# carlosnatalino/optical-rl-gym

Measured on AMD Instinct MI355X. Metric: env-steps/sec RMSA-v0 NSFNET batch 65536, higher is better.
Workload: dtype u64 bitmaps + f64 statistics

## Files before the change

optical_rl_gym_amd/csrc/orl_device_split.h:

```cpp
#pragma once
#include "orl_device_g8.h"

namespace orl {
namespace sp {

#define ORL_PROF_SLOTS 48
#define ORL_PROF_WAVES 16384
#ifdef ORL_TIMING
struct Prof { long long t; unsigned long long acc[ORL_PROF_SLOTS]; };
static __device__ unsigned long long g_prof[ORL_PROF_WAVES * ORL_PROF_SLOTS];
#define ORL_PROF_BEGIN_() do { for (int k_ = 0; k_ < ORL_PROF_SLOTS; k_++) prof.acc[k_] = 0; prof.t = clock64(); } while (0)
#define ORL_PROF_(k) do { long long n_ = clock64(); prof.acc[k] += (unsigned long long)(n_ - prof.t); prof.t = n_; } while (0)
#define ORL_PROF_END_() do { if ((threadIdx.x & 63) == 0) { const size_t w_ = ((size_t)blockIdx.x * (blockDim.x >> 6) + (threadIdx.x >> 6)) % ORL_PROF_WAVES; \
    unsigned long long* g_ = ::orl::sp::g_prof + w_ * ORL_PROF_SLOTS; \
    for (int k_ = 0; k_ < ORL_PROF_SLOTS; k_++) g_[k_] += prof.acc[k_]; } } while (0)
#define ORL_PROF_BEGIN() ORL_PROF_BEGIN_()
#define ORL_PROF_END() ORL_PROF_END_()
#define ORL_PROFA(k) ORL_PROF_(k)
#define ORL_PROF(k) ORL_PROF_(16 + (k))
#define ORL_PROFR(k) ORL_PROF_(32 + (k))
#else
struct Prof { long long t; };
#define ORL_PROF_BEGIN() do { } while (0)
#define ORL_PROF_END() do { } while (0)
#define ORL_PROFA(k) do { } while (0)
#define ORL_PROF(k) do { } while (0)
#define ORL_PROFR(k) do { } while (0)
#endif
#define ORL_PROFA_BEGIN() do { } while (0)
#define ORL_PROFA_END() do { } while (0)
#define ORL_PROFR_BEGIN() do { } while (0)
#define ORL_PROFR_END() do { } while (0)

struct Recip { double d, r; };
__device__ __forceinline__ Recip recip_of(double d) {
  Recip k;
  k.d = d;
  double r = __builtin_amdgcn_rcp(d);
  double e = __builtin_fma(-d, r, 1.0);
  r = __builtin_fma(r, e, r);
  e = __builtin_fma(-d, r, 1.0);
  k.r = __builtin_fma(r, e, r);
  return k;
}
__device__ __forceinline__ double div_by(double x, const Recip& k) {
  const double q = x * k.r;
  return __builtin_fma(__builtin_fma(-k.d, q, x), k.r, q);
}
__device__ __forceinline__ double div_pos(double x, double d) { return div_by(x, recip_of(d)); }

#include "orl_diag.h"
using g8::EnvG;
using g8::gballot;
using g8::gget;

struct Item { ulonglong2 a, b; };
__device__ __forceinline__ Item make_item(i64 env, u32 link, int nmask, u64 m0, u64 m1, u64 cores, int op) {
  Item it;
  it.a.x = (u64)(u32)env | ((u64)(link & 0xffu) << 32) | ((u64)(u32)nmask << 40) | ((u64)(u32)op << 44);
  it.a.y = m0;
  it.b.x = m1;
  it.b.y = cores;
  return it;
}
__device__ __forceinline__ void item_store(ulonglong2* q, size_t idx, const Item& it) { q[2 * idx] = it.a; q[2 * idx + 1] = it.b; }

__device__ __forceinline__ size_t wave_reserve(const DevParams& P, int cnt, u32* wave_counts, int lane) {
  const int grp = lane >> 3;
  int pre = 0, tot = 0;
#pragma unroll
  for (int g = 0; g < 8; g++) {
    const int c = __builtin_amdgcn_readlane(cnt, 8 * g);
    pre += (g < grp) ? c : 0;
    tot += c;
  }
  const size_t wave = (size_t)blockIdx.x * (blockDim.x >> 6) + (threadIdx.x >> 6);
  if (lane == 0) wave_counts[wave] = (u32)tot;
  return wave * (size_t)P.q_wave + (size_t)pre;
}

struct Mask2 { u64 lo, hi; int w0; };
__device__ __forceinline__ Mask2 mask2(int s0, int n) {
  Mask2 m;
  const int b = s0 & 63;
  const u64 ones = (1ull << n) - 1ull;
  m.w0 = s0 >> 6;
  m.lo = ones << b;
  m.hi = (b + n > 64) ? (ones >> (64 - b)) : 0ull;
  return m;
}
__device__ __forceinline__ u64 mask2_word(const Mask2& m, int w) { return (w == m.w0) ? m.lo : ((w == m.w0 + 1) ? m.hi : 0ull); }
__device__ __forceinline__ void row_apply_mask(u64* row, int s0, int n, bool provision) {
  const Mask2 m = mask2(s0, n);
  if (provision) {
    __hip_atomic_fetch_and(row + m.w0, ~m.lo, __ATOMIC_RELAXED, __HIP_MEMORY_SCOPE_WORKGROUP);
    if (m.hi) __hip_atomic_fetch_and(row + m.w0 + 1, ~m.hi, __ATOMIC_RELAXED, __HIP_MEMORY_SCOPE_WORKGROUP);
  } else {
    __hip_atomic_fetch_or(row + m.w0, m.lo, __ATOMIC_RELAXED, __HIP_MEMORY_SCOPE_WORKGROUP);
    if (m.hi) __hip_atomic_fetch_or(row + m.w0 + 1, m.hi, __ATOMIC_RELAXED, __HIP_MEMORY_SCOPE_WORKGROUP);
  }
}
template <bool CP> struct SinkEntryOf { typedef SinkEntry type; };
template <> struct SinkEntryOf<true> { typedef SinkEntryC type; };
#define ORL_EV_META(S0, N, T, PROV) ((u64)(u32)(S0) | ((u64)(u32)(N) << 9) | ((u64)(u32)(T) << 15) | ((u64)((PROV) ? 1u : 0u) << 24))
template <bool CP, bool RD = false> struct SinkT {
  typedef typename SinkEntryOf<CP>::type Entry;
  ulonglong2* ev;
  double ev_clock;
  int ev_at;
  int ev_rel0;
  int ev_t;
  unsigned short* list;
  u32* list_n;
  Entry* tab;
  u32* tally;
  int tw;
  unsigned short* mtab;
  int nrel;
  u64* rows;
  int roww;
  bool active;
  bool deferred;
  int cnt;
};
typedef SinkT<false> Sink;
__device__ __forceinline__ void sink_entry_clear(SinkEntry& t) { t.crn = 0ull; }
__device__ __forceinline__ void sink_entry_clear(SinkEntryC& t) { t.bits = 0u; }
__device__ __forceinline__ int sink_entry_add(SinkEntry* t, u64 m, int core, bool prov) {
  const u64 crn = t->crn | (prov ? (1ull << 44) : 0ull);
  const int j = (int)((crn >> 40) & 15);
  if (j < 4) t->mk0 = (j == 0 ? 0ull : t->mk0) | (m << (16 * j));
  else t->mk1 = (j == 4 ? 0ull : t->mk1) | (m << (16 * (j - 4)));
  t->crn = (crn & ((1ull << 44) | 0xffffffffffull)) | ((u64)(u32)core << (5 * j)) | ((u64)(u32)(j + 1) << 40);
  return j | (int)((crn >> 44) & 1) << 8;
}
template <bool CP, bool RD>
__device__ __forceinline__ void sink_add(SinkT<CP, RD>& s, const PathRec& rec, int core, int s0, int n, int lane, bool prov = false) {
  const int hops = path_rec_byte(rec, 0);
  if constexpr (RD) {
    u32 lm0 = 0u, lm1 = 0u;
    for (int h = lane & 7; h < hops; h += 8) {
      const int link = path_rec_byte(rec, 2 + h);
      row_apply_mask(s.rows + (size_t)link * s.roww, s0, n, prov);
      if (link < 32) lm0 |= 1u << link; else lm1 |= 1u << (link - 32);
    }
    lm0 |= (u32)dpp_i<ORL_DPP_XOR1>((int)lm0); lm1 |= (u32)dpp_i<ORL_DPP_XOR1>((int)lm1);
    lm0 |= (u32)dpp_i<ORL_DPP_XOR2>((int)lm0); lm1 |= (u32)dpp_i<ORL_DPP_XOR2>((int)lm1);
    lm0 |= (u32)dpp_i<ORL_DPP_HALF_MIRROR>((int)lm0); lm1 |= (u32)dpp_i<ORL_DPP_HALF_MIRROR>((int)lm1);
    if ((lane & 7) == 0) {
      s.ev[2 * s.ev_at] = make_ulonglong2(ORL_EV_META(s0, n, s.ev_t, prov), (u64)lm0 | ((u64)lm1 << 32));
      s.ev[2 * s.ev_at + 1] = make_ulonglong2((u64)__double_as_longlong(s.ev_clock), 0ull);
    }
  } else if constexpr (CP) {
    const int k = prov ? 0 : ++s.nrel;
    if ((lane & 7) == 0) s.mtab[k] = (unsigned short)((u32)s0 | ((u32)n << 9));
    for (int h = lane & 7; h < hops; h += 8) {
      const int link = path_rec_byte(rec, 2 + h);
      atomicOr(&s.tab[link].bits, 1u << k);
      if (s.rows) row_apply_mask(s.rows + (size_t)link * s.roww, s0, n, prov);
    }
  } else {
    const u64 m = (u64)(u32)s0 | ((u64)(u32)n << 9);
    for (int h = lane & 7; h < hops; h += 8) {
      const int r = sink_entry_add(s.tab + path_rec_byte(rec, 2 + h), m, core, prov);
      const int j = r & 15;
      s.cnt += (j == 0) ? 1 : 0;
      if (s.list && (j == 0 || (j == 1 && (r >> 8))))
        s.list[atomicAdd(s.list_n, 1u)] = (unsigned short)((j << 15) | (((lane >> 3) & 7) << 8) | path_rec_byte(rec, 2 + h));
    }
  }
}

__device__ __forceinline__ void emit_items(const DevParams& P, i64 env, const Sink& sink, bool any, int lane, ulonglong2* q, u32* counts) {
  const int gl = lane & 7, E = P.E;
  const int cnt = g8_sum(any ? sink.cnt : 0);
  const size_t base = wave_reserve(P, cnt, counts, lane);
  if (cnt) {
    size_t at = base;
    for (int l0 = 0; l0 < E; l0 += 8) {
      const int l = l0 + gl;
      const u64 crn = (l < E) ? sink.tab[l].crn : 0ull;
      const int nm = (int)((crn >> 40) & 15);
      const u32 fb = gballot(nm > 0, lane);
      if (nm > 0)
        item_store(q, at + __popc(fb & ((1u << gl) - 1u)),
                   make_item(env, (u32)l, nm, sink.tab[l].mk0, nm > 4 ? sink.tab[l].mk1 : 0ull, crn & 0xffffffffffull,
                             1 | (int)((crn >> 44) & 1) << 1));
      at += __popc(fb);
    }
  }
}

#define ORL_SVC_WIN 12
struct SvcBuf {
  double q, ht;
  u32 pk;
  int cnt;
};
__device__ __forceinline__ bool svc_empty(const SvcBuf& b) { return (b.cnt & 0xff) >= (b.cnt >> 8); }
struct SvcNext { double q, ht; u32 pk; };
__device__ __forceinline__ SvcNext svc_take(SvcBuf& b, int lane) {
  const int k = b.cnt & 0xff;
  SvcNext s;
  s.q = gget(b.q, k, lane);
  s.ht = gget(b.ht, k, lane);
  s.pk = gget(b.pk, k, lane);
  b.cnt += 1;
  return s;
}
__device__ __forceinline__ int svc_wrap(int i) { const u32 u = (u32)i, d = u - 624u; return (int)(d < u ? d : u); }
__device__ __forceinline__ int svc_choice(const double* cum, int n, double u) {
  const double x = u * (cum[n - 1] + 0.0);
  const int m = n - 1;
  if (m <= 0) return 0;
  int b = 0;
  if (m > 8 && m <= 72) {
    double p[8];
#pragma unroll
    for (int j = 0; j < 8; j++) p[j] = cum[8 * j + 7 < m ? 8 * j + 7 : m - 1];
#pragma unroll
    for (int j = 0; j < 8; j++) b += (8 * j + 7 < m && p[j] <= x) ? 1 : 0;
  } else if (m > 72) {
    int lo = 0, hi = m;
    while (lo < hi) {
      const int mid = (lo + hi) >> 1;
      if (cum[mid] <= x) lo = mid + 1; else hi = mid;
    }
    return lo;
  }
  double c[8];
#pragma unroll
  for (int k = 0; k < 8; k++) c[k] = cum[8 * b + k < m ? 8 * b + k : m - 1];
  int cnt = 8 * b;
#pragma unroll
  for (int k = 0; k < 8; k++) cnt += (8 * b + k < m && c[k] <= x) ? 1 : 0;
  return cnt;
}
template <int ENV>
__device__ __forceinline__ void svc_generate(const DevParams& P, u64* rec, u32* mt, const double2* rates_wave, int lane, int n_want,
                                             SvcBuf& sb, bool active) {
  const int gl = lane & 7;
  const bool seek = (ENV != ENV_RWA) && P.bit_rate_mode == 0;
  const int FIXED = (ENV == ENV_RWA) ? 8 : (P.bit_rate_mode == 0 ? 8 : 10);
  const u32 sh = 32u - (u32)P.rand_bits, rn = (u32)P.rand_n;
  const u64 idw = active ? rec[SC_ID_MTPOS] : 0ull;
  const int pos = (int)(idw >> 32);
  u32 cur[ORL_SVC_WIN], nxt[ORL_SVC_WIN], far[ORL_SVC_WIN];
#pragma unroll
  for (int k = 0; k < ORL_SVC_WIN; k++) {
    const int i0 = svc_wrap(pos + gl + 8 * k);
    cur[k] = active ? mt[i0] : 0u;
    nxt[k] = active ? mt[svc_wrap(i0 + 1)] : 0u;
    far[k] = active ? mt[svc_wrap(i0 + 397)] : 0u;
  }
  u32 nx[ORL_SVC_WIN];
  u32 acc0 = 0u, acc1 = 0u, acc2 = 0u;
#pragma unroll
  for (int k = 0; k < ORL_SVC_WIN; k++) {
    const u32 y = (cur[k] & 0x80000000u) | (nxt[k] & 0x7fffffffu);
    nx[k] = far[k] ^ (y >> 1) ^ ((y & 1u) ? 0x9908b0dfu : 0u);
    if (seek) {
      u32 t = cur[k];
      t ^= (t >> 11);
      t ^= (t << 7) & 0x9d2c5680u;
      t ^= (t << 15) & 0xefc60000u;
      t ^= (t >> 18);
      const u32 byte = gballot((t >> sh) < rn, lane);
      if (k < 4) acc0 |= byte << (8 * (k & 3));
      else if (k < 8) acc1 |= byte << (8 * (k & 3));
      else acc2 |= byte << (8 * (k & 3));
    }
  }
  int o = 0, my_o = 0, my_a = 0, got = 0;
  {
    const u64 m_lo = (u64)acc0 | ((u64)acc1 << 32);
    bool ok = active;
#pragma unroll
    for (int j = 0; j < 8; j++) {
      if (ok && j < n_want) {
        const int c = o + FIXED;
        int a = c - 1;
        if (seek) {
          const u64 xl = (c < 64) ? (m_lo >> c) : 0ull;
          const u32 xh = (c <= 64) ? acc2 : ((c < 8 * ORL_SVC_WIN) ? ((acc2 >> (c - 64)) << (c - 64)) : 0u);
          if (xl == 0ull && xh == 0u) ok = false;
          else a = (xl != 0ull) ? c + (int)__builtin_ctzll(xl) : 64 + (int)__builtin_ctz(xh);
        } else if (c > 8 * ORL_SVC_WIN) {
          ok = false;
        }
        if (ok) {
          if (gl == j) { my_o = o; my_a = a; }
          o = seek ? a + 1 : c;
          got = j + 1;
        }
      }
    }
  }
  const bool mine = active && gl < got;
  u32 w[10], wa = 0u;
#pragma unroll
  for (int t = 0; t < 10; t++) w[t] = (mine && t < FIXED) ? mt[svc_wrap(pos + my_o + t)] : 0u;
  if (seek && mine) wa = mt[svc_wrap(pos + my_a)];
#pragma unroll
  for (int k = 0; k < ORL_SVC_WIN; k++)
// ... 685 lines not shown
      int nd = 0, top = -1, h0 = 0x7fffffff, h1 = 0x7fffffff;
      const int hwm = e.ev_hwm;
      for (int base = gl, ord = 0; base < hwm; base += 8 * ORL_SCAN_BATCH, ord += ORL_SCAN_BATCH) {
        double tt[ORL_SCAN_BATCH];
#pragma unroll
        for (int k = 0; k < ORL_SCAN_BATCH; k++) {
          const int i = base + 8 * k;
          tt[k] = e.ev_time[i < hwm ? i : hwm - 1];
        }
        scan_batch_fence(tt);
#pragma unroll
        for (int k = 0; k < ORL_SCAN_BATCH; k++) {
          const int i = base + 8 * k;
          tt[k] = (i < hwm) ? tt[k] : INF;
        }
#pragma unroll
        for (int k = 0; k < ORL_SCAN_BATCH; k++) {
          const double t = tt[k];
          const int i = base + 8 * k;
          const bool due_t = t <= e.now;
          nd += due_t ? 1 : 0;
          const bool empty = (t == INF);
          top = empty ? top : i;
          h1 = (empty && h0 != 0x7fffffff && h1 == 0x7fffffff) ? i : h1;
          h0 = (empty && h0 == 0x7fffffff) ? i : h0;
          u32 q = (u32)__builtin_fmax(__builtin_fmin((t - e.now) * 4096.0 + 524288.0, 8388606.0), 0.0);
          q = empty ? 8388607u : q;
          q = (due_t && q > 524287u) ? 524287u : q;
          u32 x = (q << 8) | (u32)(ord + k);
#pragma unroll
          for (int j = 0; j <= NS; j++) {
            const u32 lo = kb[j] < x ? kb[j] : x;
            x = kb[j] < x ? x : kb[j];
            kb[j] = lo;
          }
        }
      }
      double bt[NS];
      int bi[NS];
#pragma unroll
      for (int k = 0; k < NS; k++) {
        const bool any = (kb[k] >> 8) < 8388607u;
        bi[k] = gl + 8 * (int)(kb[k] & 255u);
        bt[k] = any ? e.ev_time[bi[k]] : INF;
      }
      const u32 qn = kb[NS] >> 8;
      const double T_lane = (qn >= 8388607u) ? INF : (qn < 2u ? -INF : e.now + ((double)qn - 524290.0) * (1.0 / 4096.0));
      const double T = g8::g8_min(T_lane);
#pragma unroll
      for (int k = 0; k < NS; k++) { st[k] = (bt[k] < T || bt[k] <= e.now) ? bt[k] : INF; si[k] = bi[k]; }
      e.t_soon = T;
      dirty = (1 << NS) - 1;
      due_all = g8_sum(nd);
      e.ev_hwm = g8_max(top) + 1;
      {
        const bool v0 = h0 < e.ev_hwm, v1 = h1 < e.ev_hwm;
        const u32 b0 = gballot(v0, lane), b1 = gballot(v1, lane);
        unsigned short* fs = (unsigned short*)(e.scal + SC_FREE0);
        if (v0) fs[__popc(b0 & ((1u << gl) - 1u))] = (unsigned short)h0;
        if (v1) fs[__popc(b0) + __popc(b1 & ((1u << gl) - 1u))] = (unsigned short)h1;
        e.nfree = __popc(b0) + __popc(b1);
      }
      ORL_PROF(5);
    }
    int ndl = 0;
    double ct = INF;
    int ci = 0x7fffffff, ck = 0;
#pragma unroll
    for (int k = 0; k < NS; k++) {
      const bool due = st[k] <= e.now;
      ndl += due ? 1 : 0;
      if (due && (st[k] < ct || (st[k] == ct && si[k] < ci))) { ct = st[k]; ci = si[k]; ck = k; }
    }
    const int tot = g8_sum(ndl);
    if (tot == 0) {
      if (e.now < e.t_soon) break;
      if (round > 0 || due_all >= 0) {
        if (!sink.active) { ORL_DBG(8, 1); ORL_DBG(9, e.now < e.t_soon ? 0 : 1); ORL_DBG(10, due_all > 0 ? 1 : 0); sink.deferred = true; return; }
        break;
      }
      continue;
    }
    if (!sink.active) {
      const int total = due_all >= 0 ? due_all : tot;
      if constexpr (CP) {
        sink.active = total <= P.rel_limit;
      } else {
      sink.active = total + extra <= P.item_masks;
      if (!sink.active && total < 200) {
        for (int base = gl; base < e.ev_hwm; base += 64) {
          double tt[8];
#pragma unroll
          for (int k = 0; k < 8; k++) {
            const int i = base + 8 * k;
            const double v = e.ev_time[i < e.ev_hwm ? i : e.ev_hwm - 1];
            tt[k] = (i < e.ev_hwm) ? v : INF;
          }
#pragma unroll
          for (int k = 0; k < 8; k++) {
            if (tt[k] <= e.now) {
              const u64 info = e.ev_info[base + 8 * k];
              const PathRec rec = path_rec_load(P, (int)(info & 0xffffffu));
              const int hops = path_rec_byte(rec, 0);
              for (int h = 0; h < hops; h++) {
                const int link = path_rec_byte(rec, 2 + h);
                atomicAdd(sink.tally + (link >> 2), 1u << (8 * (link & 3)));
              }
            }
          }
        }
        wave_fence();
        u32 mx = 0;
        for (int wd = gl; wd < sink.tw; wd += 8) {
          const u32 v = sink.tally[wd];
          const u32 a0 = v & 0xff, a1 = (v >> 8) & 0xff, a2 = (v >> 16) & 0xff, a3 = v >> 24;
          u32 m01 = a0 > a1 ? a0 : a1, m23 = a2 > a3 ? a2 : a3;
          m01 = m01 > m23 ? m01 : m23;
          mx = mx > m01 ? mx : m01;
        }
        sink.active = g8_max((int)mx) <= P.item_masks;
      }
      }
      if (!sink.active) {
        ORL_DBG(11, 1);
        sink.deferred = true;
        return;
      }
    }
    if constexpr (CP) {
      u32 rk = 0u;
      int n_round = 0;
      if (e.rank_pairs && __ballot(ndl > 1) == 0ull) {
        int r = 1;
#define ORL_RANK_STEP(OT, OI) { const double ot_ = (OT); const int oi_ = (OI); \
                                r += (ot_ < ct || (ot_ == ct && oi_ < ci)) ? 1 : 0; \
                                if (ot_ < INF && gl == (oi_ & 7)) e.ev_time[oi_] = INF; }
        ORL_RANK_STEP(dpp_d<ORL_DPP_XOR1>(ct), dpp_i<ORL_DPP_XOR1>(ci))
        ORL_RANK_STEP(dpp_d<ORL_DPP_XOR2>(ct), dpp_i<ORL_DPP_XOR2>(ci))
        ORL_RANK_STEP(dpp_d<ORL_DPP_XOR3>(ct), dpp_i<ORL_DPP_XOR3>(ci))
        {
          const double mt = dpp_d<ORL_DPP_HALF_MIRROR>(ct);
          const int mi = dpp_i<ORL_DPP_HALF_MIRROR>(ci);
          ORL_RANK_STEP(mt, mi)
          ORL_RANK_STEP(dpp_d<ORL_DPP_XOR1>(mt), dpp_i<ORL_DPP_XOR1>(mi))
          ORL_RANK_STEP(dpp_d<ORL_DPP_XOR2>(mt), dpp_i<ORL_DPP_XOR2>(mi))
          ORL_RANK_STEP(dpp_d<ORL_DPP_XOR3>(mt), dpp_i<ORL_DPP_XOR3>(mi))
        }
#undef ORL_RANK_STEP
        n_round = tot;
        if (ndl == 1) {
          if (gl == (ci & 7)) e.ev_time[ci] = INF;
          rk = (u32)r << (6 * ck);
          dirty |= 1 << ck;
#pragma unroll
          for (int k = 0; k < NS; k++)
            if (k == ck) st[k] = INF;
        }
      } else {
        for (;;) {
          double bt = ct;
          int bi = ci, bl = gl;
#define ORL_MIN_STEP(CTRL) { double ot = dpp_d<CTRL>(bt); int oi = dpp_i<CTRL>(bi); int ol = dpp_i<CTRL>(bl); \
                             if (ot < bt || (ot == bt && oi < bi)) { bt = ot; bi = oi; bl = ol; } }
          ORL_MIN_STEP(ORL_DPP_XOR1) ORL_MIN_STEP(ORL_DPP_XOR2) ORL_MIN_STEP(ORL_DPP_HALF_MIRROR)
#undef ORL_MIN_STEP
          if (!(bt <= e.now)) break;
          n_round++;
          if (gl == (bi & 7)) e.ev_time[bi] = INF;
          if (gl == bl) {
            rk |= (u32)n_round << (6 * ck);
            dirty |= 1 << ck;
            ct = INF; ci = 0x7fffffff;
            int nk = 0;
#pragma unroll
            for (int k = 0; k < NS; k++) {
              if (k == ck) st[k] = INF;
              const bool due = st[k] <= e.now;
              if (due && (st[k] < ct || (st[k] == ct && si[k] < ci))) { ct = st[k]; ci = si[k]; nk = k; }
            }
            ck = nk;
          }
        }
      }
      ORL_PROF(6);
      int d_br = 0, d_nh = 0;
      const int nfree0 = e.nfree, nrel0 = sink.nrel;
      unsigned short* fs = (unsigned short*)(e.scal + SC_FREE0);
      while (rk) {
        const int k = (int)__builtin_ctz(rk) / 6;
        const int r = (int)((rk >> (6 * k)) & 63u);
        rk &= ~(63u << (6 * k));
        int idx = si[0];
#pragma unroll
        for (int j = 1; j < NS; j++) idx = (k == j) ? si[j] : idx;
        const u64 info = (idx == pushed_idx) ? pushed_info : ((idx == pre_idx) ? pre_info : e.ev_info[idx]);
        const PathRec rec = path_rec_load(P, (int)(info & 0xffffffu));
        const int s0 = (int)((info >> 24) & 0xfffu), n = (int)((info >> 36) & 0xffu), br = (int)((info >> 49) & 0x7fffu);
        const int hops = path_rec_byte(rec, 0), kk = nrel0 + r;
        if constexpr (RD) {
          u64 lm = 0ull;
          for (int h = 0; h < hops; h++) {
            const int link = path_rec_byte(rec, 2 + h);
            row_apply_mask(sink.rows + (size_t)link * sink.roww, s0, n, false);
            lm |= 1ull << link;
          }
          sink.ev[2 * (sink.ev_rel0 + kk - 1)] = make_ulonglong2(ORL_EV_META(s0, n, sink.ev_t, false), lm);
          sink.ev[2 * (sink.ev_rel0 + kk - 1) + 1] = make_ulonglong2((u64)__double_as_longlong(e.now), 0ull);
        } else {
        sink.mtab[kk] = (unsigned short)((u32)s0 | ((u32)n << 9));
        for (int h = 0; h < hops; h++) {
          const int link = path_rec_byte(rec, 2 + h);
          atomicOr(&sink.tab[link].bits, 1u << kk);
          if (sink.rows) row_apply_mask(sink.rows + (size_t)link * sink.roww, s0, n, false);
        }
        }
        const int fp = nfree0 + r - 1;
        if (fp < ORL_FREE_SLOTS) fs[fp] = (unsigned short)idx;
        d_br += br;
        d_nh += n * hops;
      }
      e.ev_cnt -= n_round;
      e.nfree = (nfree0 + n_round < ORL_FREE_SLOTS) ? nfree0 + n_round : ORL_FREE_SLOTS;
      sink.nrel = nrel0 + n_round;
      e.s_br -= (i64)g8_sum(d_br);
      e.s_nh -= (i64)g8_sum(d_nh);
    } else {
      u64 inf0 = 0;
      PathRec rc0 = PathRec();
      if (ci != 0x7fffffff) { inf0 = (ci == pushed_idx) ? pushed_info : ((ci == pre_idx) ? pre_info : e.ev_info[ci]); rc0 = path_rec_load(P, (int)(inf0 & 0xffffffu)); }
      ORL_PROF(6);
      for (;;) {
        double bt = ct;
        int bi = ci, bl = gl;
  #define ORL_MIN_STEP(CTRL) { double ot = dpp_d<CTRL>(bt); int oi = dpp_i<CTRL>(bi); int ol = dpp_i<CTRL>(bl); \
                               if (ot < bt || (ot == bt && oi < bi)) { bt = ot; bi = oi; bl = ol; } }
        ORL_MIN_STEP(ORL_DPP_XOR1) ORL_MIN_STEP(ORL_DPP_XOR2) ORL_MIN_STEP(ORL_DPP_HALF_MIRROR)
  #undef ORL_MIN_STEP
        if (!(bt <= e.now)) break;
        const u64 info = gget(inf0, bl, lane);
        PathRec rec;
        rec.q[0] = gget(rc0.q[0], bl, lane); rec.q[1] = gget(rc0.q[1], bl, lane);
        rec.q[2] = gget(rc0.q[2], bl, lane); rec.q[3] = gget(rc0.q[3], bl, lane);
        if (gl == (bi & 7)) e.ev_time[bi] = INF;
        if (gl == bl) {
          dirty |= 1 << ck;
          ct = INF; ci = 0x7fffffff;
          int nk = 0;
  #pragma unroll
          for (int k = 0; k < NS; k++) {
            if (k == ck) st[k] = INF;
            const bool due = st[k] <= e.now;
            if (due && (st[k] < ct || (st[k] == ct && si[k] < ci))) { ct = st[k]; ci = si[k]; nk = k; }
          }
          ck = nk;
          if (ci != 0x7fffffff) { inf0 = (ci == pushed_idx) ? pushed_info : ((ci == pre_idx) ? pre_info : e.ev_info[ci]); rc0 = path_rec_load(P, (int)(inf0 & 0xffffffu)); }
        }
        const int s0 = (int)((info >> 24) & 0xfffu), n = (int)((info >> 36) & 0xffu);
        const int core = (int)((info >> 44) & 0x1fu), br = (int)((info >> 49) & 0x7fffu);
        e.ev_cnt--;
        g8::free_push(e, gl, bi);
        sink_add(sink, rec, core, s0, n, lane);
        e.s_br -= br;
        e.s_nh -= (i64)n * path_rec_byte(rec, 0);
      }
    }
    ORL_PROF(7);
    if (e.now < e.t_soon) break;
  }
  {
    double m = st[0];
#pragma unroll
    for (int k = 1; k < NS; k++) m = st[k] < m ? st[k] : m;
    const double lm = g8::g8_min(m);
    e.next_rel = lm < e.t_soon ? lm : e.t_soon;
  }
  out.dirty = dirty;
#pragma unroll
  for (int k = 0; k < NS; k++) { out.t[k] = st[k]; out.i[k] = si[k]; }
  ORL_PROF(8);
}

template <int ENV, int W>
__device__ __forceinline__ void rel_serial(const DevParams& P, i64 env, int lane) {
  u64* s = P.scal + env * ORL_SCAL_WORDS;
  if (!((s[SC_ACC] >> 16) & 1ull)) return;
  const int gl = lane & 7;
  if (gl == 0) atomicAdd(P.q_stat, 1u);
  EnvG e;
  g8::env_load(P, e, env);
  if (P.pipeline2) e.rs = e.cs + 2 * P.C;
  g8::release_due<ENV, W>(P, e, lane);
  e.t_soon = -__builtin_inf();
  if (gl == 0) {
    s[SC_ACC] = s[SC_ACC] & ~(1ull << 16);
    s[SC_NEXTREL] = (u64)__double_as_longlong(e.next_rel);
    s[SC_TSOON] = (u64)__double_as_longlong(e.t_soon);
    s[SC_SBR] = (u64)e.s_br;
    s[SC_SNH] = (u64)e.s_nh;
    s[SC_EV] = pack2(e.ev_hwm, e.ev_cnt);
    s[SC_HINT] = pack2(e.nfree, 0);
  }
}

template <int W, bool CACHED = false>
__device__ __forceinline__ void row_stat_lane(const u64 (&a)[W], int S, RowStat& st, int& max_empty, int& edge, u32* cache = nullptr,
                                              u32 touched = 0u, bool update = false) {
  int nu = 0, lo = 1 << 20, hi = 0, free_ = 0, nf = 0, best = 0, c = 0;
  u64 inter[CACHED ? W : 1];
#pragma unroll
  for (int w = 0; w < W; w++) {
    const u64 maskw = word_mask_lo(S - 64 * w);
    const u64 used = ~a[w] & maskw;
    const u64 prev_top = (w == 0) ? 0ull : (a[w - 1] >> 63);
    const u64 carry_u = (w == 0) ? 0ull : (prev_top ^ 1ull);
    nu += __popcll(used & ~((used << 1) | carry_u));
    if (used) {
      const int l = 64 * w + (int)__builtin_ctzll(used);
      lo = l < lo ? l : lo;
      hi = 64 * w + 64 - (int)__builtin_clzll(used);
    }
    free_ += __popcll(a[w]);
    if (CACHED) {
      const u64 na = ~a[w];
      const bool full = na == 0ull;
      const int lead = full ? 64 : (int)__builtin_ctzll(na), trail = full ? 64 : (int)__builtin_clzll(na);
      best = (c + lead) > best ? (c + lead) : best;
      c = full ? c + 64 : trail;
      inter[CACHED ? w : 0] = full ? 0ull : ((a[w] & (a[w] + 1ull)) & (~0ull >> trail));
    } else if (a[w] == ~0ull) {
      c += 64;
      best = c > best ? c : best;
    } else {
      const int lead = (int)__builtin_ctzll(~a[w]);
      const int inner = word_longest_run_flat(a[w]);
      const int cand = (c + lead) > inner ? (c + lead) : inner;
      best = cand > best ? cand : best;
      c = (int)__builtin_clzll(~a[w]);
    }
  }
  if (CACHED) {
    best = c > best ? c : best;
    u32 cw = *cache;
    u32 need = touched;
#pragma unroll
    for (int w = 0; w < W; w++) {
      const int f = (int)((cw >> (6 * w)) & 63u);
      if (!((touched >> w) & 1u)) {
        if (f == 63) need |= 1u << w;
        else best = f > best ? f : best;
      }
    }
    while (need) {
      const int w = (int)__builtin_ctz(need);
      need &= need - 1u;
      u64 x = inter[0];
#pragma unroll
      for (int k = 1; k < (CACHED ? W : 1); k++) x = (w == k) ? inter[k] : x;
      const int f = word_longest_run_flat(x);
      best = f > best ? f : best;
      cw = (cw & ~(63u << (6 * w))) | ((u32)f << (6 * w));
    }
    if (update) *cache = cw;
  }
  const bool two = nu > 1;
  const int fb = two ? nu - 1 : 0;
  max_empty = best;
  const int tw = (S - 1) >> 6, tb = (S - 1) & 63;
  int top_bit = 0;
#pragma unroll
  for (int w = 0; w < W; w++) top_bit = (w == tw) ? (int)((a[w] >> tb) & 1ull) : top_bit;
  edge = (int)(a[0] & 1ull) + top_bit;
  nf = nu - 1 + edge;
  st.nu = nu; st.lo = lo; st.hi = hi; st.occ = two ? hi - lo : 0; st.fb = fb; st.free_ = free_; st.nf = nf;
}

struct RowInc { int free_, nu, lo, hi, me; };
template <int W> __device__ __forceinline__ u64 row_word(const u64 (&a)[W], int w) {
  u64 x = 0ull;
#pragma unroll
  for (int k = 0; k < W; k++) x = (w == k) ? a[k] : x;
  return x;
}
template <int W> __device__ __forceinline__ int row_run_below(const u64 (&a)[W], int p) {
  int len = 0;
  for (int q = p; q > 0; q -= 64) {
    const int wq = q >> 6, b = q & 63;
    const u64 hi = row_word<W>(a, wq), lo = row_word<W>(a, wq - 1);
    const u64 x = (b == 0) ? lo : ((hi << (64 - b)) | (lo >> b));
    const int c = (x == ~0ull) ? 64 : (int)__builtin_clzll(~x);
    len += c;
    if (c < 64) break;
  }
  return len;
}
template <int W> __device__ __forceinline__ int row_run_from(const u64 (&a)[W], int p) {
  int len = 0;
  for (int q = p; q < 64 * W; q += 64) {
    const int wq = q >> 6, b = q & 63;
    const u64 lo = row_word<W>(a, wq), hi = row_word<W>(a, wq + 1);
    const u64 x = (b == 0) ? lo : ((lo >> b) | (hi << (64 - b)));
    const int c = (x == ~0ull) ? 64 : (int)__builtin_ctzll(~x);
    len += c;
    if (c < 64) break;
  }
  return len;
}
template <int W> __device__ __forceinline__ int row_longest_free(const u64 (&a)[W]) {
  int best = 0, c = 0;
#pragma unroll
  for (int w = 0; w < W; w++) {
    if (a[w] == ~0ull) {
      c += 64;
    } else {
      const int lead = (int)__builtin_ctzll(~a[w]), trail = (int)__builtin_clzll(~a[w]);
      const int inner = word_longest_run_flat((a[w] & (a[w] + 1ull)) & (~0ull >> trail));
      const int cand = (c + lead) > inner ? (c + lead) : inner;
      best = cand > best ? cand : best;
      c = trail;
    }
  }
  return c > best ? c : best;
}
template <int W>
__device__ __forceinline__ void row_inc_apply(u64 (&a)[W], int S, int s0, int n, bool prov, RowInc& s) {
  const int l = row_run_below<W>(a, s0), r = row_run_from<W>(a, s0 + n);
  const int joins = ((s0 > 0 && l == 0) ? 1 : 0) + ((s0 + n < S && r == 0) ? 1 : 0);
  const Mask2 mm = mask2(s0, n);
#pragma unroll
  for (int w = 0; w < W; w++) a[w] ^= mask2_word(mm, w);
  if (prov) {
    s.free_ -= n;
    s.nu += 1 - joins;
    s.lo = s0 < s.lo ? s0 : s.lo;
    s.hi = s0 + n > s.hi ? s0 + n : s.hi;
    if (l + n + r == s.me) s.me = row_longest_free<W>(a);
  } else {
    s.free_ += n;
    s.nu -= 1 - joins;
    const int m = l + n + r;
    s.me = m > s.me ? m : s.me;
    if (s.nu == 0) { s.lo = 1 << 20; s.hi = 0; }
    else {
      if (s0 == s.lo) s.lo = s0 + n + r;
      if (s0 + n == s.hi) s.hi = s0 - l;
    }
  }
}

template <int W>
__device__ __forceinline__ u32 row_inner_cache(const u64* row) {
  u32 cw = 0u;
#pragma unroll
  for (int w = 0; w < (W <= 5 ? W : 0); w++) {
    const u64 a = row[w];
    int f = 0;
    if (a != ~0ull) {
      const int lead = (int)__builtin_ctzll(~a), trail = (int)__builtin_clzll(~a);
      f = word_longest_run(a & ~word_range(0, lead) & ~word_range(64 - trail, 64));
    }
    cw |= (u32)f << (6 * w);
  }
  return cw;
}
__device__ __forceinline__ u32 mask_words(int s0, int n) { return (1u << (s0 >> 6)) | (1u << ((s0 + n - 1) >> 6)); }
template <int W>
__device__ __forceinline__ void row_occ_fb(const u64 (&a)[W], int S, int& occ, int& fb) {
  int nu = 0, lo = 1 << 20, hi = 0;
#pragma unroll
  for (int w = 0; w < W; w++) {
    const u64 used = ~a[w] & word_mask_lo(S - 64 * w);
    const u64 carry_u = (w == 0) ? 0ull : ((a[w > 0 ? w - 1 : 0] >> 63) ^ 1ull);
    nu += __popcll(used & ~((used << 1) | carry_u));
    if (used) {
      const int l = 64 * w + (int)__builtin_ctzll(used);
      lo = l < lo ? l : lo;
      hi = 64 * w + 64 - (int)__builtin_clzll(used);
    }
  }
  const bool two = nu > 1;
  occ = two ? hi - lo : 0;
  fb = two ? nu - 1 : 0;
}

template <int ENV, int W, bool EARLY = false>
__device__ __forceinline__ void row_item_lane1(const DevParams& P, const Wmem& M, const i64 env, const int link, const u32 bits,
                                               const unsigned short* mtab, int second, Prof& prof, bool early_ls = false,
                                               double* stash_env = nullptr, u32* sig = nullptr, u32 sig_val = 0u) {
  const int E = P.E, S = P.S;
  const int nmask = __popc(bits);
  const bool prov_first = (bits & 1u) != 0;
  const bool shared = prov_first && nmask >= 2;
  const bool role_b = shared && second;
  const bool role_a = shared && !second;
  u64* row = wm_bm(P, M, env) + (size_t)link * W;
  int* cs = wm_cs(P, M, env);
  int* rs = cs + 2;
  double* ls = wm_ls(P, M, env) + 4 * link;
  const double now = M.clk ? M.clk[2 * (env - M.clk_env0) + 1] : __longlong_as_double((i64)wm_scal(P, M, env)[SC_NOW]);
  const double now_prov = M.clk ? M.clk[2 * (env - M.clk_env0)] : __longlong_as_double((i64)wm_scal(P, M, env)[SC_NOWA]);
  double2 ls01 = make_double2(0.0, 0.0), ls23 = make_double2(0.0, 0.0);
  if (early_ls && !role_b) { ls01 = *(const double2*)ls; ls23 = *(const double2*)(ls + 2); }
  u32* ocg = (ENV != ENV_RWA && !M.oc0 && M.ocg) ? M.ocg + (env - M.cenv0) * E + link : nullptr;
  u32 ocg_v = 0u;
  if (ocg && !role_b) ocg_v = *ocg;
  u64 a[W];
#pragma unroll
  for (int w = 0; w < W; w++) a[w] = row[w];
  ORL_PROFR(3);
  u64 fin[EARLY ? W : 1];
  u32 later_e = 0u, mw0_e = 0u, mwf_e = 0u;
  if constexpr (EARLY) {
    u32 rest_e = bits & (bits - 1u);
    int first_e = (int)__builtin_ctz(bits);
    if (role_b) { first_e = (int)__builtin_ctz(rest_e); rest_e &= rest_e - 1u; }
    if (role_a) rest_e = 0u;
#pragma unroll
    for (int w = 0; w < W; w++) fin[w] = a[w];
    for (u32 r = bits & ~1u; r; r &= r - 1u) {
      const int k = (int)__builtin_ctz(r);
      const u32 mw = mtab[k];
      const int s0 = (int)(mw & 0x1ff), n = (int)(mw >> 9);
      if (k == first_e) mwf_e = mw;
      if ((rest_e >> k) & 1u) later_e |= mask_words(s0, n);
      const Mask2 mm = mask2(s0, n);
#pragma unroll
      for (int w = 0; w < W; w++) a[w] &= ~mask2_word(mm, w);
    }
    if (bits & 1u) {
      mw0_e = mtab[0];
      if (first_e == 0) mwf_e = mw0_e;
      const Mask2 mm = mask2((int)(mw0_e & 0x1ff), (int)(mw0_e >> 9));
#pragma unroll
      for (int w = 0; w < W; w++) a[w] |= mask2_word(mm, w);
    }
    rw_release_lds();
    if (sig) __hip_atomic_store(sig, sig_val, __ATOMIC_RELAXED, __HIP_MEMORY_SCOPE_WORKGROUP);
    ORL_PROFR(9);
  }
  u32 rest = bits & (bits - 1u);
  int first = (int)__builtin_ctz(bits);
  u32 touched = 0u;
  if (role_b) {
    const u32 mw = EARLY ? mw0_e : (u32)mtab[0];
    const int s0 = (int)(mw & 0x1ff), n = (int)(mw >> 9);
    touched = mask_words(s0, n);
    const Mask2 mm = mask2(s0, n);
#pragma unroll
    for (int w = 0; w < W; w++) a[w] &= ~mask2_word(mm, w);
    first = (int)__builtin_ctz(rest);
    rest &= rest - 1u;
  }
  if (role_a) rest = 0u;
  u32* ocw = (ENV != ENV_RWA && M.oc0) ? M.oc0 + (env - M.cenv0) * E + link : nullptr;
  int occ0 = 0, fb0 = 0;
  if (ENV != ENV_RWA) {
    if (ocg) { }
    else if (!ocw) row_occ_fb<W>(a, S, occ0, fb0);
    else if (!role_b) { const u32 c = *ocw; occ0 = (int)(c >> 16); fb0 = (int)(c & 0xffffu); }
  }
  const bool rel_f = first != 0;
  {
    const u32 mw = EARLY ? mwf_e : (u32)mtab[first];
    const int s0 = (int)(mw & 0x1ff), n = (int)(mw >> 9);
    touched |= mask_words(s0, n);
    const Mask2 mm = mask2(s0, n);
#pragma unroll
    for (int w = 0; w < W; w++) {
      const u64 m = mask2_word(mm, w);
      a[w] = rel_f ? (a[w] | m) : (a[w] & ~m);
    }
  }
  ORL_PROFR(4);
  RowStat after;
  int max_empty = 0, edge = 0;
  u32* icw = (ENV != ENV_RWA && M.ic0) ? M.ic0 + (env - M.cenv0) * E + link : nullptr;
  if (ENV != ENV_RWA) {
#ifdef ORL_DIAG_INSTEAD_OF_ROW_SUMMARY
    ORL_DIAG_INSTEAD_OF_ROW_SUMMARY
#else
    if (W >= 3 && W <= 5 && icw) row_stat_lane<W, (W >= 3 && W <= 5)>(a, S, after, max_empty, edge, icw, touched, !role_a);
    else row_stat_lane<W>(a, S, after, max_empty, edge);
#endif
  } else {
    int f = 0;
#pragma unroll
    for (int w = 0; w < W; w++) f += __popcll(a[w]);
    after.free_ = f;
  }
  ORL_PROFR(5);
  const int free_ = after.free_;
  const double cur_util = div_pos((double)(S - free_), (double)S);
  double cur_frag = 0.0, cur_comp = 0.0;
  if (ENV != ENV_RWA && free_ > 0) {
    int me = (after.nf > 1 && !(after.nf == 2 && edge == 2)) ? max_empty : 0;
    cur_frag = 1.0 - div_pos((double)me, (double)free_);
    if (after.nu > 1) cur_comp = div_pos((double)(after.hi - after.lo), (double)(S - free_)) * div_pos(1.0, (double)after.nu);
    else cur_comp = 1.0;
  }
  if (ocw && role_a) *ocw = ((u32)after.occ << 16) | (u32)after.fb;
  const double clock = rel_f ? now : now_prov;
  const int n_rest = __popc(rest);
#ifdef ORL_DIAG_NO_SECOND_ROUND
  const u64 any_b = 0ull;
#else
  const u64 any_b = __ballot(role_b);
#endif
  for (int round = 0; round < 2; round++) {
    if (round == 1 && !any_b) break;
    if ((round == 1) == role_b) {
      if (role_b || !early_ls) { ls01 = *(const double2*)ls; ls23 = *(const double2*)(ls + 2); }
      double last_update = ls23.y;
      double util = ls01.x, frag = ls01.y, comp = ls23.x;
      if (stash_env && rel_f) { stash_env[2 * link] = util; stash_env[2 * link + 1] = comp; }
#ifdef ORL_DIAG_NO_F64
      if (false) {
#else
      if (clock > 0) {
#endif
        const double time_diff = clock - last_update;
        const Recip rc = recip_of(clock);
        util = div_by((util * last_update) + (cur_util * time_diff), rc);
        if (ENV != ENV_RWA) {
          frag = div_by((frag * last_update) + (cur_frag * time_diff), rc);
          comp = div_by((comp * last_update) + (cur_comp * time_diff), rc);
        }
      }
      last_update = clock;
      if (now > 0 && n_rest > 0) {
        const Recip rn = recip_of(now);
        for (int k = 0; k < n_rest; k++) {
          util = div_by((util * now) + 0.0, rn);
          if (ENV != ENV_RWA) { frag = div_by((frag * now) + 0.0, rn); comp = div_by((comp * now) + 0.0, rn); }
        }
      }
      *(double2*)ls = make_double2(util, frag);
      *(double2*)(ls + 2) = make_double2(comp, last_update);
    }
    wave_fence();
  }
  ORL_PROFR(6);
  if (ocw && role_b) { const u32 c = *ocw; occ0 = (int)(c >> 16); fb0 = (int)(c & 0xffffu); }
  int occL = after.occ, fbL = after.fb;
  if (rest) {
    u32 later = 0u;
    if constexpr (EARLY) {
      later = later_e;
#pragma unroll
      for (int w = 0; w < W; w++) a[w] = fin[w];
    } else {
      for (u32 r = rest; r; r &= r - 1u) {
        const u32 mw = mtab[__builtin_ctz(r)];
        const int s0 = (int)(mw & 0x1ff), n = (int)(mw >> 9);
        later |= mask_words(s0, n);
        const Mask2 mm = mask2(s0, n);
#pragma unroll
        for (int w = 0; w < W; w++) a[w] |= mask2_word(mm, w);
      }
    }
    if (ENV != ENV_RWA) row_occ_fb<W>(a, S, occL, fbL);
    if (icw) {
      u32 cw = *icw;
#pragma unroll
      for (int w = 0; w < (W <= 5 ? W : 0); w++) cw |= ((later >> w) & 1u) ? (63u << (6 * w)) : 0u;
      *icw = cw;
    }
  }
  if (ENV != ENV_RWA) {
    if (ocg) { occ0 = (int)(ocg_v >> 16); fb0 = (int)(ocg_v & 0xffffu); }
    if (ocg && shared) {
      if (role_a) { atomicAdd(cs, -occ0); atomicAdd(cs + 1, -fb0); atomicAdd(rs, -after.occ); atomicAdd(rs + 1, -after.fb); }
      else { atomicAdd(cs, occL); atomicAdd(cs + 1, fbL); atomicAdd(rs, occL); atomicAdd(rs + 1, fbL); }
    } else {
      const int d_occ = occL - occ0, d_fb = fbL - fb0;
      if (d_occ) atomicAdd(cs, d_occ);
      if (d_fb) atomicAdd(cs + 1, d_fb);
      if (rel_f) {
        if (d_occ) atomicAdd(rs, d_occ);
        if (d_fb) atomicAdd(rs + 1, d_fb);
      }
    }
  }
  if (!role_a) {
    if constexpr (!EARLY) {
#pragma unroll
      for (int w = 0; w < W; w++) row[w] = a[w];
    }
    if (ocw) *ocw = ((u32)occL << 16) | (u32)fbL;
    if (ocg) *ocg = ((u32)occL << 16) | (u32)fbL;
  }
  ORL_PROFR(7);
}

template <int ENV, int W>
__device__ __forceinline__ void row_item_lane(const DevParams& P, const Wmem& M, const Item it, Prof& prof) {
  constexpr bool MIXED = true;
  const int E = P.E, S = P.S;
  const i64 env = (i64)(u32)it.a.x;
  const int link = (int)((it.a.x >> 32) & 0xff), nmask = (int)((it.a.x >> 40) & 15);
  const bool release = ((it.a.x >> 44) & 1) != 0;
  const bool prov_first = MIXED && ((it.a.x >> 45) & 1) != 0;
  const u64 cores = it.b.y;
  u64* bm = wm_bm(P, M, env);
  int* cs = wm_cs(P, M, env);
  int* rs = MIXED ? cs + 2 * P.C : nullptr;
  double* ls = wm_ls(P, M, env);
  const double now = M.clk ? M.clk[2 * (env - M.clk_env0) + 1] : __longlong_as_double((i64)wm_scal(P, M, env)[SC_NOW]);
  const double now_prov = M.clk ? M.clk[2 * (env - M.clk_env0)] : __longlong_as_double((i64)wm_scal(P, M, env)[SC_NOWA]);
  const double2 ls01 = *(const double2*)(ls + 4 * link), ls23 = *(const double2*)(ls + 4 * link + 2);
  double last_update = ls23.y;
  double util = ls01.x, frag = ls01.y, comp = ls23.x;
  ORL_PROFR(3);
  u64 a[W];
  int pk = 0, prev_core = -1;
  for (int k = 0; k < nmask; k++) {
    const int core = (int)((cores >> (5 * k)) & 0x1f);
    const u64 mw = k < 4 ? (it.a.y >> (16 * k)) : (it.b.x >> (16 * (k - 4)));
    const int s0 = (int)(mw & 0x1ff), n = (int)((mw >> 9) & 0x7f);
    const bool rel_k = MIXED ? !(k == 0 && prov_first) : release;
    const double clock = (MIXED && !rel_k) ? now_prov : now;
    const bool first_at_clock = (k == 0) || (MIXED && k == 1 && prov_first);
    u64* row = bm + (size_t)(core * E + link) * W;
    if (core != prev_core) {
#pragma unroll
      for (int w = 0; w < W; w++) a[w] = row[w];
      if (ENV != ENV_RWA) {
        int occ_b, fb_b;
        row_occ_fb<W>(a, S, occ_b, fb_b);
        pk = (occ_b << 16) | fb_b;
      }
      prev_core = core;
    }
    {
      const Mask2 mm = mask2(s0, n);
#pragma unroll
      for (int w = 0; w < W; w++) {
        const u64 m = mask2_word(mm, w);
        a[w] = rel_k ? (a[w] | m) : (a[w] & ~m);
        if (m) row[w] = a[w];
      }
    }
    RowStat after;
    int max_empty = 0, edge = 0;
    ORL_PROFR(4);
    if (ENV != ENV_RWA) {
      row_stat_lane<W>(a, S, after, max_empty, edge);
      ORL_PROFR(5);
      const int d_occ = after.occ - (pk >> 16), d_fb = after.fb - (pk & 0xffff);
      pk = (after.occ << 16) | after.fb;
      if (d_occ) atomicAdd(cs + 2 * core, d_occ);
      if (d_fb) atomicAdd(cs + 2 * core + 1, d_fb);
      if (MIXED && rel_k) {
        if (d_occ) atomicAdd(rs + 2 * core, d_occ);
        if (d_fb) atomicAdd(rs + 2 * core + 1, d_fb);
      }
    } else {
      int f = 0;
#pragma unroll
      for (int w = 0; w < W; w++) f += __popcll(a[w]);
      after.free_ = f;
    }
    if (clock > 0) {
      if (first_at_clock) {
        const double time_diff = clock - last_update;
        const int free_ = after.free_;
        const Recip rc = recip_of(clock);
        double cur_util = div_pos((double)(S - free_), (double)S);
        util = div_by((util * last_update) + (cur_util * time_diff), rc);
        if (ENV != ENV_RWA) {
          double cur_frag = 0.0, cur_comp = 0.0;
          if (free_ > 0) {
            int me = (after.nf > 1 && !(after.nf == 2 && edge == 2)) ? max_empty : 0;
            cur_frag = 1.0 - div_pos((double)me, (double)free_);
            if (after.nu > 1) cur_comp = div_pos((double)(after.hi - after.lo), (double)(S - free_)) * div_pos(1.0, (double)after.nu);
            else cur_comp = 1.0;
          }
          frag = div_by((frag * last_update) + (cur_frag * time_diff), rc);
          comp = div_by((comp * last_update) + (cur_comp * time_diff), rc);
        }
      } else {
        const Recip rc = recip_of(clock);
        util = div_by((util * clock) + 0.0, rc);
        if (ENV != ENV_RWA) { frag = div_by((frag * clock) + 0.0, rc); comp = div_by((comp * clock) + 0.0, rc); }
      }
    }
    last_update = clock;
  }
  ORL_PROFR(6);
  *(double2*)(ls + 4 * link) = make_double2(util, frag);
  *(double2*)(ls + 4 * link + 2) = make_double2(comp, last_update);
  ORL_PROFR(7);
}

}
}
```

Measured before the change: 1.535 billion.

## Incrementally update cached per-word inner free-run lengths instead of recomputing

Adds an O(1) incremental update of the cached per-word longest interior free run on allocate/release, and falls back to a full search only when the cached maximum may be invalidated. Lanes also share cached words across the pair via a DPP lane shuffle instead of each recomputing them, and later releases update the cache in place rather than marking words dirty. This removes repeated word_longest_run_flat scans in the per-step row statistics. The cost is more branching and more complex cache invariants across roles, which could introduce subtle correctness risk.

```diff
diff --git a/optical_rl_gym_amd/csrc/orl_device_split.h b/optical_rl_gym_amd/csrc/orl_device_split.h
--- a/optical_rl_gym_amd/csrc/orl_device_split.h
+++ b/optical_rl_gym_amd/csrc/orl_device_split.h
@@ -1,5 +1,6 @@
 #pragma once
 #include "orl_device_g8.h"
+#include "orl_inner_update.h"
 
 namespace orl {
 namespace sp {
@@ -1291,11 +1292,10 @@
   }
 }
 
-template <int W, bool CACHED = false>
-__device__ __forceinline__ void row_stat_lane(const u64 (&a)[W], int S, RowStat& st, int& max_empty, int& edge, u32* cache = nullptr,
-                                              u32 touched = 0u, bool update = false) {
+template <int W, bool CACHED, bool UPD>
+__device__ __forceinline__ void row_stat_core(const u64 (&a)[W], int S, RowStat& st, int& max_empty, int& edge, const u32* cache, u32 arg,
+                                              bool rel_f, u32& cw, u32& skip, int& rounds) {
   int nu = 0, lo = 1 << 20, hi = 0, free_ = 0, nf = 0, best = 0, c = 0;
-  u64 inter[CACHED ? W : 1];
 #pragma unroll
   for (int w = 0; w < W; w++) {
     const u64 maskw = word_mask_lo(S - 64 * w);
@@ -1315,7 +1315,6 @@
       const int lead = full ? 64 : (int)__builtin_ctzll(na), trail = full ? 64 : (int)__builtin_clzll(na);
       best = (c + lead) > best ? (c + lead) : best;
       c = full ? c + 64 : trail;
-      inter[CACHED ? w : 0] = full ? 0ull : ((a[w] & (a[w] + 1ull)) & (~0ull >> trail));
     } else if (a[w] == ~0ull) {
       c += 64;
       best = c > best ? c : best;
@@ -1329,27 +1328,58 @@
   }
   if (CACHED) {
     best = c > best ? c : best;
-    u32 cw = *cache;
-    u32 need = touched;
+    cw = *cache;
+    u32 need = arg;
+    skip = 0u;
+    if (UPD) {
+      const int s0 = (int)(arg & 0x1ffu), n = (int)((arg >> 9) & 0x7fu);
+      const u32 prov_b = arg >> 16;
+      const int wa = s0 >> 6, wb = wa + 1, e1 = (s0 & 63) + n - 64;
+      need = 1u << wa;
+      u32 mine = need;
+      if (e1 > 0) {
+        const int sh = 6 * wb, f0 = (int)((cw >> sh) & 63u);
+        u64 x = a[0];
+#pragma unroll
+        for (int k = 1; k < W; k++) x = (wb == k) ? a[k] : x;
+        int f = orl_inner_update(x, 0, e1, rel_f, f0);
+        f = (f0 == 63 || ((prov_b >> wb) & 1u)) ? ORL_INNER_SEARCH : f;
+        cw = (cw & ~(63u << sh)) | ((u32)f << sh);
+        mine |= 1u << wb;
+#ifdef ORL_TIMING
+        if (f == ORL_INNER_SEARCH) rounds += 0x10000;
+#endif
+      }
+      if (lane_id() != 0) skip = prov_b & ~mine;
+      else need |= prov_b;
+    }
+    const u32 given = need | skip;
 #pragma unroll
     for (int w = 0; w < W; w++) {
       const int f = (int)((cw >> (6 * w)) & 63u);
-      if (!((touched >> w) & 1u)) {
+      if (!((given >> w) & 1u)) {
         if (f == 63) need |= 1u << w;
         else best = f > best ? f : best;
       }
     }
+#ifdef ORL_TIMING
+    if (UPD && (need & ~((1u << ((arg & 0x1ffu) >> 6)) | (arg >> 16)))) rounds += 0x100;
+#endif
     while (need) {
+      rounds++;
       const int w = (int)__builtin_ctz(need);
       need &= need - 1u;
-      u64 x = inter[0];
-#pragma unroll
-      for (int k = 1; k < (CACHED ? W : 1); k++) x = (w == k) ? inter[k] : x;
+      u64 x = a[0];
+#pragma unroll
+      for (int k = 1; k < W; k++) x = (w == k) ? a[k] : x;
+      const u64 nx = ~x;
+      const bool full = nx == 0ull;
+      const int trail = full ? 0 : (int)__builtin_clzll(nx);
+      x = full ? 0ull : ((x & (x + 1ull)) & (~0ull >> trail));
       const int f = word_longest_run_flat(x);
       best = f > best ? f : best;
       cw = (cw & ~(63u << (6 * w))) | ((u32)f << (6 * w));
     }
-    if (update) *cache = cw;
   }
   const bool two = nu > 1;
   const int fb = two ? nu - 1 : 0;
@@ -1361,6 +1391,14 @@
   edge = (int)(a[0] & 1ull) + top_bit;
   nf = nu - 1 + edge;
   st.nu = nu; st.lo = lo; st.hi = hi; st.occ = two ? hi - lo : 0; st.fb = fb; st.free_ = free_; st.nf = nf;
+}
+template <int W, bool CACHED = false>
+__device__ __forceinline__ void row_stat_lane(const u64 (&a)[W], int S, RowStat& st, int& max_empty, int& edge, u32* cache = nullptr,
+                                              u32 touched = 0u, bool update = false) {
+  u32 cw = 0u, skip = 0u;
+  int rounds = 0;
+  row_stat_core<W, CACHED, false>(a, S, st, max_empty, edge, cache, touched, false, cw, skip, rounds);
+  if (CACHED && update) *cache = cw;
 }
 
 struct RowInc { int free_, nu, lo, hi, me; };
@@ -1528,11 +1566,11 @@
   }
   u32 rest = bits & (bits - 1u);
   int first = (int)__builtin_ctz(bits);
-  u32 touched = 0u;
+  u32 prov_b = 0u;
   if (role_b) {
     const u32 mw = EARLY ? mw0_e : (u32)mtab[0];
     const int s0 = (int)(mw & 0x1ff), n = (int)(mw >> 9);
-    touched = mask_words(s0, n);
+    prov_b = mask_words(s0, n);
     const Mask2 mm = mask2(s0, n);
 #pragma unroll
     for (int w = 0; w < W; w++) a[w] &= ~mask2_word(mm, w);
@@ -1548,10 +1586,12 @@
     else if (!role_b) { const u32 c = *ocw; occ0 = (int)(c >> 16); fb0 = (int)(c & 0xffffu); }
   }
   const bool rel_f = first != 0;
+  u32* icw = (ENV != ENV_RWA && M.ic0) ? M.ic0 + (env - M.cenv0) * E + link : nullptr;
+  u32 stat_arg;
   {
     const u32 mw = EARLY ? mwf_e : (u32)mtab[first];
     const int s0 = (int)(mw & 0x1ff), n = (int)(mw >> 9);
-    touched |= mask_words(s0, n);
+    stat_arg = mw | (prov_b << 16);
     const Mask2 mm = mask2(s0, n);
 #pragma unroll
     for (int w = 0; w < W; w++) {
@@ -1562,13 +1602,29 @@
   ORL_PROFR(4);
   RowStat after;
   int max_empty = 0, edge = 0;
-  u32* icw = (ENV != ENV_RWA && M.ic0) ? M.ic0 + (env - M.cenv0) * E + link : nullptr;
   if (ENV != ENV_RWA) {
 #ifdef ORL_DIAG_INSTEAD_OF_ROW_SUMMARY
     ORL_DIAG_INSTEAD_OF_ROW_SUMMARY
 #else
-    if (W >= 3 && W <= 5 && icw) row_stat_lane<W, (W >= 3 && W <= 5)>(a, S, after, max_empty, edge, icw, touched, !role_a);
-    else row_stat_lane<W>(a, S, after, max_empty, edge);
+    if (W >= 3 && W <= 5 && icw) {
+      int rounds = 0;
+      u32 cw, skip;
+      row_stat_core<W, (W >= 3 && W <= 5), true>(a, S, after, max_empty, edge, icw, stat_arg, rel_f, cw, skip, rounds);
+      {
+        const u32 cwa = (u32)__builtin_amdgcn_update_dpp(0, (int)cw, 0x138 , 0xf, 0xf, false);
+        const int s_lo = 6 * (int)__builtin_ctz(skip | 32u), s_hi = 6 * (31 - (int)__builtin_clz(skip | 1u));
+        const u32 m = skip ? ((63u << s_lo) | (63u << s_hi)) : 0u;
+        cw = (cw & ~m) | (cwa & m);
+        const int f_lo = (int)(((cwa & m) >> s_lo) & 63u), f_hi = (int)(((cwa & m) >> s_hi) & 63u);
+        const int f = f_lo > f_hi ? f_lo : f_hi;
+        max_empty = f > max_empty ? f : max_empty;
+      }
+      if (!role_a) *icw = cw;
+#ifdef ORL_TIMING
+      prof.acc[44] += 1; prof.acc[45] += __ballot((rounds & 0xff) >= 2) != 0ull; prof.acc[46] += __ballot((rounds & 0xff) >= 2 && (rounds & 0xff00)) != 0ull;
+      prof.acc[47] += __ballot((rounds & 0xff) >= 2 && (rounds >> 16)) != 0ull;
+#endif
+    } else row_stat_lane<W>(a, S, after, max_empty, edge);
 #endif
   } else {
     int f = 0;
@@ -1632,6 +1688,7 @@
   int occL = after.occ, fbL = after.fb;
   if (rest) {
     u32 later = 0u;
+    u32 cw = icw ? *icw : 0u;
     if constexpr (EARLY) {
       later = later_e;
 #pragma unroll
@@ -1640,7 +1697,15 @@
       for (u32 r = rest; r; r &= r - 1u) {
         const u32 mw = mtab[__builtin_ctz(r)];
         const int s0 = (int)(mw & 0x1ff), n = (int)(mw >> 9);
-        later |= mask_words(s0, n);
+        if (W >= 3 && W <= 5 && icw) {
+          const int wa = s0 >> 6, b = s0 & 63, e = b + n, sh = 6 * wa;
+          if (e > 64) later |= (1u << wa) | (2u << wa);
+          else {
+            const int f0 = (int)((cw >> sh) & 63u);
+            const int f = orl_inner_update(row_word<W>(a, wa), b, e, true, f0);
+            cw = (f0 == 63) ? cw : ((cw & ~(63u << sh)) | ((u32)f << sh));
+          }
+        } else later |= mask_words(s0, n);
         const Mask2 mm = mask2(s0, n);
 #pragma unroll
         for (int w = 0; w < W; w++) a[w] |= mask2_word(mm, w);
@@ -1648,7 +1713,6 @@
     }
     if (ENV != ENV_RWA) row_occ_fb<W>(a, S, occL, fbL);
     if (icw) {
-      u32 cw = *icw;
 #pragma unroll
       for (int w = 0; w < (W <= 5 ? W : 0); w++) cw |= ((later >> w) & 1u) ? (63u << (6 * w)) : 0u;
       *icw = cw;
diff --git a/optical_rl_gym_amd/csrc/orl_inner_update.h b/optical_rl_gym_amd/csrc/orl_inner_update.h
--- /dev/null
+++ b/optical_rl_gym_amd/csrc/orl_inner_update.h
@@ -0,0 +1,26 @@
+#pragma once
+#include <stdint.h>
+
+#if defined(__HIPCC__)
+#define ORL_INNER_FN __host__ __device__ __forceinline__
+#else
+#define ORL_INNER_FN static inline
+#endif
+
+#define ORL_INNER_SEARCH 63
+
+ORL_INNER_FN int orl_inner_update(uint64_t x, int b, int e, bool release, int f0) {
+  const int L = b == 0 ? 0 : (int)__builtin_clzll(~(x << (64 - b)));
+  const int R = e == 64 ? 0 : (int)__builtin_ctzll(~(x >> e));
+  const bool low_edge = L == b, high_edge = R == 64 - e;
+  const int cl = low_edge ? 0 : L, cr = high_edge ? 0 : R;
+  const bool inner_run = !low_edge && !high_edge;
+  const int m = L + (e - b) + R;
+  const int side = cl > cr ? cl : cr;
+  if (release) {
+    if (inner_run) return m > f0 ? m : f0;
+    return ((cl > 0 && cl == f0) || (cr > 0 && cr == f0)) ? ORL_INNER_SEARCH : f0;
+  }
+  if (inner_run && m == f0) return ORL_INNER_SEARCH;
+  return side > f0 ? side : f0;
+}
```

After: 1.522 billion. No clear change (-0.8%).
